# wicstas/pine

Hardware: AMD Instinct MI355X
Metric: Msamples/s (higher is better)
Workload: dtype f32

## Files before the change

pine_amd/csrc/pine_kernels.hip:

```cpp
#include <hip/hip_runtime.h>

#include <climits>
#include <cmath>
#include <cstring>
#include <deque>

#include "pine_plan.h"
#include "pine_bvh_build_device.h"
#include "pine_embree_order.h"
#include "../data/rcpps_table.h"
namespace pine_gpu {

static int device_build(std::vector<BuildPrim>& prims, const std::vector<BuildTask>& roots, FlatAccel& A, int device) {
  int ndev = 0;
  if (hipGetDeviceCount(&ndev) != hipSuccess || device < 0 || device >= ndev) {
    (void)hipGetLastError();
    return -1;
  }
  if (hipSetDevice(device) != hipSuccess) return -1;
  const size_t n = prims.size();
  BuildPrim *d_prims = nullptr, *d_scratch = nullptr;
  BuildTask *d_tasks[2] = {nullptr, nullptr};
  BuildDecision* d_dec = nullptr;
  int *d_rank = nullptr, *d_perm = nullptr, *d_src = nullptr, *d_counts = nullptr;
// ... 203 lines not shown
        } else if (cnt < 0 || ch < 0 || ch >= n_nodes) return bad("child index");
        else todo.push_back({ch, depth + 1});
      }
    }
  }
  for (int i = 0; i < A.top_prim_begin; i++) {
    int tri;
    memcpy(&tri, &A.tri_leaf[size_t(i) * 12 + 9], 4);
    if (tri < 0 || tri >= n_tris) return bad("triangle index of a leaf record");
  }
  for (int i = A.top_prim_begin; i < n_prims; i++)
    if (A.prims[size_t(i)] < 0 || A.prims[size_t(i)] >= int(shapes.size())) return bad("geometry index of a top-level primitive");
  for (const DShape& sh : shapes) {
    if (sh.material < 0 || size_t(sh.material) >= num_materials) return bad("material index");
    if (sh.kind == SHAPE_MESH) {
      int first, count, bvh;
      memcpy(&first, &sh.f[0], 4), memcpy(&count, &sh.f[1], 4), memcpy(&bvh, &sh.f[2], 4);
      if (count > 0 && (bvh < 1 || bvh >= int(A.bvhs.size()) || first < 0 || first + count > n_tris)) return bad("mesh record");
    }
  }
  for (const DLight& L : lights)
    if (L.kind == LIGHT_AREA && (L.geom < 0 || L.geom >= int(shapes.size()))) return bad("area light geometry");
  return 0;
}

}

using namespace pine_gpu;

enum : int { kSpecSourceNone = 0, kSpecSourceCache = 1, kSpecSourceCompiledHere = 2, kSpecSourceBackground = 3 };

namespace pine_gpu {
AbiFingerprint abi_fingerprint() {
  return AbiFingerprint{sizeof(DeviceScene), sizeof(WorkParams), sizeof(Counters), sizeof(DNode), sizeof(DShape), sizeof(DMaterial), sizeof(DLight),
                        offsetof(WorkParams, total_items), offsetof(DeviceScene, cam), kQFields, kQWinDwords, int(QC_WORDS), kQTokenDwords,
                        kTravRecordDwords, kQCtxGlobalDwordsPlain, kQCtxGlobalDwordsSss};
}
}

struct LoadedKernel {
  int device = 0;
  std::string key, image;
  hipModule_t module = nullptr;
  hipFunction_t fn = nullptr;
  ~LoadedKernel() {
    if (module) {
      int keep = 0;
      (void)hipGetDevice(&keep);
      (void)hipSetDevice(device);
      (void)hipModuleUnload(module);
      (void)hipSetDevice(keep);
    }
  }
};
struct LoadedKernels {
  static constexpr size_t kMaxLoaded = 16;
  std::mutex mu;
  std::deque<std::shared_ptr<LoadedKernel>> recent;
  static LoadedKernels& get() {
    static LoadedKernels* q = new LoadedKernels();
    return *q;
  }
  std::shared_ptr<LoadedKernel> find(int device, const std::string& key) {
    std::lock_guard<std::mutex> lock(mu);
    for (auto& k : recent)
      if (k->device == device && k->key == key) return k;
    return nullptr;
  }
  void remember(const std::shared_ptr<LoadedKernel>& k) {
    std::lock_guard<std::mutex> lock(mu);
    recent.push_front(k);
    if (recent.size() > kMaxLoaded) recent.pop_back();
  }
  void forget(const std::string& key) {
    std::lock_guard<std::mutex> lock(mu);
    for (auto it = recent.begin(); it != recent.end();)
      it = (*it)->key == key ? recent.erase(it) : it + 1;
  }
};

constexpr int kUnset = INT_MIN;
struct PlanKnobs {
  int specialize, lds_tris, xstage, trav_min_lanes, trav_min_trips, max_pixels, fair_period, pool_items;
  bool specialize_force, no_lds_scene, mega, no_tile_classes, no_fork, ckpt_every_launch;
  double idle_budget_s;
  int pin_kind, pin_order, lds_nodes_cap;
};
static PlanKnobs read_knobs() {
  auto num = [](const char* name) { return getenv(name) ? atoi(getenv(name)) : kUnset; };
  auto set = [](const char* name) { return getenv(name) != nullptr; };
  const char* kernel = getenv("PINE_GPU_KERNEL");
  const char* budget = getenv("PINE_GPU_IDLE_BUDGET_S");
  const int ckpt = num("PINE_GPU_CKPT_EVERY_LAUNCH");
  int pin_kind = -1, pin_order = -1;
  if (const char* pin = getenv("PINE_GPU_TEST_VARIANT")) {
    const std::string s = pin;
    const size_t colon = s.find(':');
    const std::string kind = s.substr(0, colon), digits = colon == std::string::npos ? "" : s.substr(colon + 1);
    pin_kind = kind == "queue" ? 0 : kind == "mega" ? 1 : 2;
    if (digits.empty() || digits.size() > 6 || digits.find_first_not_of("0123456789") != std::string::npos) pin_kind = 2;
    else pin_order = atoi(digits.c_str());
  }
  return PlanKnobs{num("PINE_GPU_SPECIALIZE"), num("PINE_GPU_LDS_TRIS"), num("PINE_GPU_XSTAGE"), num("PINE_GPU_TRAV_MIN_LANES"),
                   num("PINE_GPU_TRAV_MIN_TRIPS"), num("PINE_GPU_MAX_PIXELS"), num("PINE_GPU_FAIR_PERIOD"), num("PINE_GPU_POOL_ITEMS"),
                   set("PINE_GPU_SPECIALIZE_FORCE"), set("PINE_GPU_NO_LDS_SCENE"), kernel && std::string(kernel) == "mega",
                   set("PINE_GPU_NO_TILE_CLASSES"), set("PINE_GPU_NO_FORK"), ckpt != kUnset && ckpt != 0,
                   budget && atof(budget) > 0 ? atof(budget) : 30.0, pin_kind, pin_order, num("PINE_GPU_TEST_LDS_NODES")};
}

static int plan_adopt_kernel(pine_gpu_plan* p, bool compile_here);
static int plan_specialize(pine_gpu_plan* p, const FlatAccel& A, const std::vector<DShape>& shapes, const std::vector<int>& packed_prims,
                           const pine_gpu_render_params* prm, unsigned need, const PlanKnobs& K) {
  if (K.pin_kind >= 0) return 0;
  bool explicit_want = (prm->flags & PINE_GPU_FLAG_SPECIALIZE) != 0;
  bool automatic = !explicit_want && !(prm->flags & PINE_GPU_FLAG_NO_SPECIALIZE);
  if (K.specialize != kUnset) {
    if (K.specialize != 0) explicit_want = true, automatic = false;
    else explicit_want = automatic = false;
  }
  if ((!explicit_want && !automatic) || p->queue_variant < 0 || (prm->flags & (PINE_GPU_FLAG_FAST | PINE_GPU_FLAG_VERTEX_LOG))) return 0;
  const PineKernelVariant& V = kQueueVariants[p->queue_variant];
  const auto t0 = std::chrono::steady_clock::now();
  const unsigned kLayout = F_LDS_SCENE | F_LDS_TOP | F_LDS_REST | F_XSTAGE | F_SSS;
  unsigned exact = (V.features & kLayout) | need;
  std::string baked;
  if (!(prm->flags & (PINE_GPU_FLAG_SPECIALIZE_NO_BAKE | PINE_GPU_FLAG_ORDER_EMBREE))) {
    if (!(V.features & F_XSTAGE) && A.top_prim_begin == 0) baked = generate_baked_scene(A, shapes, packed_prims);
    else if ((V.features & F_XSTAGE) && A.bvhs.size() == 2) baked = generate_baked_scene(A, shapes, packed_prims, true);
  }
  if (baked.empty() && exact == V.features && !K.specialize_force) return 0;
  if (!baked.empty()) exact |= F_BAKED;
  hipDeviceProp_t prop;
  HIP_OK(hipGetDeviceProperties(&prop, prm->device));
  std::string arch = prop.gcnArchName;
  if (arch.find(':') != std::string::npos) arch = arch.substr(0, arch.find(':'));
  KernelRequest& R = p->spec_request;
  R.baked = baked, R.features = exact, R.ctx = V.ctx, R.arch = arch;
  p->spec_t0 = t0;
  p->spec_explicit = explicit_want;
  std::string err;
  const int found = kernel_cache_lookup(R, err);
  if (found < 0) {
    if (!explicit_want) {
      R = KernelRequest();
      return 0;
    }
    set_error(err);
    return -1;
  }
  if (found == 1) {
    p->spec_source = kSpecSourceCache;
    if (plan_adopt_kernel(p, explicit_want && !(prm->flags & PINE_GPU_FLAG_SPECIALIZE_ASYNC)) == 0) return 0;
    if (explicit_want && !(prm->flags & PINE_GPU_FLAG_SPECIALIZE_ASYNC)) return -1;
    const bool packaged = R.packaged;
    (void)unlink(R.path.c_str());
    const int again = kernel_cache_lookup(R, err, packaged);
    if (again < 0 || (again == 1 && plan_adopt_kernel(p, false) != 0)) {
      p->spec_state.store(kSpecFailed);
      p->spec_async_error = again < 0 ? err : std::string(pine_gpu_last_error());
      return 0;
    }
    if (again == 1) return 0;
  } else if (explicit_want && !(prm->flags & PINE_GPU_FLAG_SPECIALIZE_ASYNC)) {
    p->spec_source = kSpecSourceCompiledHere;
    return plan_adopt_kernel(p, true);
  }
  p->spec_source = kSpecSourceBackground;
  p->spec_job = SpecQueue::get().submit(R, explicit_want);
  if (!p->spec_job) {
    p->spec_state.store(explicit_want ? kSpecFailed : kSpecNone);
    p->spec_async_error = "the background compile queue is full";
    return 0;
  }
  p->spec_state.store(kSpecBuilding);
  return 0;
}

static int plan_adopt_kernel(pine_gpu_plan* p, bool compile_here) {
  KernelRequest& R = p->spec_request;
  bool skip_packaged = false;
  for (int attempt = 0;; attempt++) {
    std::string err;
    const int found = kernel_cache_lookup(R, err, skip_packaged);
    if (found < 0 || (found == 0 && (!compile_here || !kernel_compile(R, err)))) {
      set_error(found == 0 && !compile_here ? "scene specialisation: the code object is not in the cache" : err);
      return -1;
    }
// ... 698 lines not shown
  W.num_local_tiles = (total_tiles - prm->shard_rank + prm->shard_world - 1) / prm->shard_world;
  W.samples_per_item = kspi;
  W.items_per_pixel = spp / kspi;
  W.log2_items_per_pixel = 0;
  while ((1 << W.log2_items_per_pixel) < W.items_per_pixel) W.log2_items_per_pixel++;
  W.tiles_x_magic = unsigned(((1ull << 32) + unsigned(W.tiles_x) - 1) / unsigned(W.tiles_x));
  W.total_items = (unsigned long long)W.num_local_tiles * W.items_per_pixel * 64ull;
  W.tile_order = nullptr;
  W.serial_tiles = 0;
  std::vector<int> serial, free_tiles;
  if (in_path_rng && !uber_rng && kernel.queued() && (kernel.features & F_SSS) != 0 && !K.no_tile_classes && !K.no_fork && spp > 1 &&
      spp_pow2 &&
      tile_classes(H, sp, W, serial, free_tiles) && !free_tiles.empty() && !serial.empty()) {
    p->tile_order = serial;
    p->tile_order.insert(p->tile_order.end(), free_tiles.begin(), free_tiles.end());
    W.serial_tiles = int(serial.size());
    W.samples_per_item = 1;
    W.items_per_pixel = spp;
    W.log2_items_per_pixel = 0;
    while ((1 << W.log2_items_per_pixel) < W.items_per_pixel) W.log2_items_per_pixel++;
    W.total_items = (unsigned long long)W.serial_tiles * 64ull + (unsigned long long)(W.num_local_tiles - W.serial_tiles) * W.items_per_pixel * 64ull;
  }
  if (p->film_w > 65535 || p->film_h > 65535) {
    set_error("film sides above 65535 are not supported");
    return -1;
  }
  W.pass_first_chunk = 0;
  W.pass_chunks = W.items_per_pixel;
  W.pass_chunks_magic = W.pass_chunks > 1 ? unsigned(((1ull << 32) + unsigned(W.pass_chunks) - 1) / unsigned(W.pass_chunks)) : 0u;
  W.pass_row_stride = spp;
  W.free_tile_base = W.serial_tiles;
  W.pass_first_serial_tile = 0;
  if (!plan_passes(W.num_local_tiles, spp, W.samples_per_item, W.serial_tiles, p->pass_samples_req, p->pass_plan)) return -1;
  const PassPlan& PP = p->pass_plan;
  for (int j = 0; j < PP.n; j++)
    if ((PP.rows(j, spp) + unsigned(PP.pass(j, spp).first_sample)) * 64ull >= (1ull << 32)) {
      set_error(PP.n > 1 ? "film pixels x samples of one pass must stay below 2^32 (fewer samples per pass, or several shards)"
                         : "film pixels x samples per pixel of one shard must stay below 2^32 (render in several shards)");
      return -1;
    }
  return 0;
}

static WorkParams pass_work(const pine_gpu_plan* p, int j) {
  WorkParams W = p->W;
  const int spp = p->S.spp;
  const PassPlan::Pass a = p->pass_plan.pass(j, spp);
  if (p->W.items_per_pixel == 1) {
    W.free_tile_base = a.first_tile;
    W.total_items = (unsigned long long)a.tiles * 64ull;
    return W;
  }
  W.serial_tiles = a.tiles;
  W.pass_first_serial_tile = a.first_tile;
  W.free_tile_base = p->W.serial_tiles;
  W.pass_first_chunk = a.first_sample / W.samples_per_item;
  W.pass_chunks = a.samples / W.samples_per_item;
  W.pass_chunks_magic = W.pass_chunks > 1 ? unsigned(((1ull << 32) + unsigned(W.pass_chunks) - 1) / unsigned(W.pass_chunks)) : 0u;
  W.pass_row_stride = a.samples;
  W.total_items = (unsigned long long)a.tiles * 64ull + (unsigned long long)p->pass_plan.free_tiles * unsigned(W.pass_chunks) * 64ull;
  if (p->W.serial_tiles > 0 && a.tiles == 0) {
    W.fork_sealed = 0;
    W.max_pixels = 1 << 20;
  }
  return W;
}

static void schedule_params(pine_gpu_plan* p, const FlatAccel& A, const pine_gpu_render_params* prm, bool uber_rng, const PlanKnobs& K) {
  WorkParams& W = p->W;
  const bool in_path_rng = p->serial_rng;
  W.idle_budget_ticks = (unsigned long long)(K.idle_budget_s * 100e6);
  W.debug_force_bail = (prm->flags & PINE_GPU_FLAG_DEBUG_FORCE_BAIL) ? 1 : 0;
  W.trav_min_lanes = (p->S.lds_nodes > 0 && size_t(p->S.lds_nodes) * 10 >= A.nodes.size() * 9) ? 48 : 0;
  W.trav_min_trips = 8;
  if (!p->spec_request.baked.empty() && (p->spec_request.features & F_XSTAGE)) W.trav_min_trips = 3;
  if (K.trav_min_lanes != kUnset) W.trav_min_lanes = K.trav_min_lanes;
  if (K.trav_min_trips != kUnset) W.trav_min_trips = K.trav_min_trips > 0 ? K.trav_min_trips : 1;
  W.fork_sealed = (in_path_rng && !uber_rng && !K.no_fork) ? 1 : 0;
  W.max_pixels = W.fork_sealed ? 320 : (1 << 20);
  if (K.max_pixels > 0) W.max_pixels = K.max_pixels;
  W.pick_spins = 8;
  W.fair_period = 8;
  if (K.fair_period != kUnset) W.fair_period = K.fair_period;
  W.pool_items = in_path_rng ? 64 : 512;
  if (K.pool_items > 0) W.pool_items = K.pool_items;
  if (W.serial_tiles > 0) W.pool_items = 64;
  W.progress = nullptr;
  W.vertex_log = nullptr;
}

static int size_and_allocate(pine_gpu_plan* p, const pine_gpu_render_params* prm, int spp, const PlanKnobs& K) {
  WorkParams& W = p->W;
  if (prm->flags & PINE_GPU_FLAG_PROGRESS) {
    HIP_OK(hipHostMalloc((void**)&p->h_progress, sizeof(unsigned long long), hipHostMallocMapped));
    *p->h_progress = 0;
    HIP_OK(hipHostGetDevicePointer((void**)&W.progress, p->h_progress, 0));
  }
  hipDeviceProp_t prop;
  HIP_OK(hipGetDeviceProperties(&prop, prm->device));
  int blocks_per_cu = 0;
  const PathKernel kernel = plan_kernel(p);
  if (kernel.queued()) {
    blocks_per_cu = 1;
    HIP_OK(hipFuncSetAttribute(kernel.fn, hipFuncAttributeMaxDynamicSharedMemorySize, int(p->lds_bytes)));
  } else {
    HIP_OK(hipOccupancyMaxActiveBlocksPerMultiprocessor(&blocks_per_cu, kernel.fn, kBlock, p->lds_bytes));
  }
  if (blocks_per_cu < 1) blocks_per_cu = 1;
  if (blocks_per_cu > 8) blocks_per_cu = 8;
  const PassPlan& PP = p->pass_plan;
  unsigned long long launch_items = 0, sample_rows = 0;
  int ckpt_chunks = 0;
  for (int j = 0; j < PP.n; j++) {
    const WorkParams Wj = pass_work(p, j);
    launch_items = std::max(launch_items, Wj.total_items);
    sample_rows = std::max(sample_rows, PP.rows(j, spp));
    ckpt_chunks = std::max(ckpt_chunks, Wj.pass_chunks);
  }
  const unsigned long long want = (launch_items + kernel.ctx - 1) / kernel.ctx;
  p->grid = int(std::min<unsigned long long>(want, (unsigned long long)prop.multiProcessorCount * blocks_per_cu));
  if (p->grid < 1) p->grid = 1;
  if (!p->serial_rng && K.pool_items == kUnset) {
    unsigned long long share = launch_items / ((unsigned long long)p->grid * 32ull);
    int claim = 512;
    while (claim < 2048 && (unsigned long long)claim * 2ull <= share) claim *= 2;
    W.pool_items = claim;
  }

  if (W.items_per_pixel > 1) {
    p->bytes_ckpt = (size_t)(W.num_local_tiles - W.serial_tiles) * ckpt_chunks * 64 * sizeof(ulonglong2);
    HIP_OK(POOL_ALLOC(p->d_ckpt, p->bytes_ckpt));
    if (PP.n > 1) {
      p->bytes_carry = (size_t)PP.free_tiles * 64 * sizeof(ulonglong2);
      HIP_OK(POOL_ALLOC(p->d_rng_carry, p->bytes_carry));
    }
  }
  if (PP.n > 1) {
    HIP_OK(POOL_ALLOC(p->d_sum, (size_t)W.num_local_tiles * 64 * sizeof(float4)));
    p->bytes_carry += (size_t)W.num_local_tiles * 64 * sizeof(float4);
  }
  p->ckpt_every_launch = K.ckpt_every_launch;
  if (!p->tile_order.empty()) {
    HIP_OK(POOL_ALLOC(p->d_tile_order, p->tile_order.size() * sizeof(int)));
    HIP_OK(hipMemcpy(p->d_tile_order, p->tile_order.data(), p->tile_order.size() * sizeof(int), hipMemcpyHostToDevice));
    W.tile_order = p->d_tile_order;
  }
  p->bytes_samples = size_t(sample_rows) * 64 * sizeof(float4);
  HIP_OK(POOL_ALLOC(p->d_samples, p->bytes_samples));
  const size_t fold_slots = size_t(p->grid) * kernel.ctx;
  HIP_OK(POOL_ALLOC(p->d_fold, size_t(prm->max_path_length) * 8 * fold_slots * sizeof(float)));
  if (kernel.queued()) {
    const size_t token_dwords = (kernel.features & F_SSS) ? size_t(p->grid) * (kernel.ctx <= 1024 ? 1024 : 2048) * kQTokenDwords : 0;
    HIP_OK(POOL_ALLOC(p->d_ctxg, (size_t(p->grid) * kernel.ctx * q_ctx_global_dwords(kernel.features) + token_dwords) * sizeof(uint32_t)));
  }
  HIP_OK(POOL_ALLOC(p->d_counters, sizeof(Counters)));
  p->timed = (prm->flags & PINE_GPU_FLAG_TIMING) != 0;
  if (p->timed)
    for (auto& slot : p->ev)
      for (auto& e : slot) HIP_OK(hipEventCreate(&e));
  return 0;
}

static int plan_build(pine_gpu_plan* p, pine_gpu_scene* scene, const pine_gpu_render_params* prm) {
  const PlanKnobs K = read_knobs();
  SceneHost& H = scene_host(scene);
  const int spp = check_params(H, prm);
// ... 566 lines not shown
```

pine_amd/csrc/pine_kernels_device.h:

```cpp
#pragma once
#include <hip/hip_runtime.h>

#include <type_traits>

#include "pine_device.h"

namespace pine_gpu {

constexpr int kBlock = 256;
constexpr int kTile = 8;
#ifndef PINE_LDS_FOLD_LEVELS
#define PINE_LDS_FOLD_LEVELS 1
#endif
constexpr int kLdsFoldLevels = PINE_LDS_FOLD_LEVELS;
constexpr int kPoolItems = 128;
constexpr int kMaxDepth = 32;
constexpr unsigned kFBoxes = F_AABB | F_OBB;
constexpr unsigned kFAnalytic = F_AABB | F_OBB | F_SPHERE | F_DISK | F_CONE | F_UBER;

#ifdef PINE_PROFILE_SECTIONS
static __device__ unsigned long long g_region_lanes[16], g_region_hits[16];
#ifndef PINE_PROFILE_REGIONS
#define REGION(id)
#else
// ... 62 lines not shown
struct SceneView {
  const DShape* leaf;
  const DShape* shapes;
  const DMaterial* materials;
  const DNode* nodes;
  const int* prims;
  const DBvh* bvhs;
  const DLight* lights;
  const float* tri_verts;
  const DNodeOp* node_ops;
  int stack_top;
  int num_shapes;
  const float4* tri_leaf;
  const float* tri_attrs;
  const DNode* lds_nodes;
  int lds_node_count;
  const uint2* lds_tri_entries;
  const float4* lds_tri_verts;
  const EmbreeNode* etree;
  int etree_root;
  const int* emesh;
  int num_emesh;
  const unsigned* rcpps;
};

typedef unsigned int u32x4 __attribute__((ext_vector_type(4)));
typedef __attribute__((address_space(3))) const u32x4 lds_u32x4;
template <unsigned F>
__device__ __forceinline__ DNode fetch_node(const SceneView& S, int index) {
  union {
    DNode n;
    u32x4 q[4];
  } b;
  if constexpr (F & F_LDS_TOP) {
    if (index < S.lds_node_count) {
      lds_u32x4* p = (lds_u32x4*)(S.lds_nodes) + size_t(index) * 4;
      b.q[0] = p[0], b.q[1] = p[1], b.q[2] = p[2], b.q[3] = p[3];
      return b.n;
    }
  }
  const u32x4* g = reinterpret_cast<const u32x4*>(S.nodes + index);
  b.q[0] = g[0], b.q[1] = g[1], b.q[2] = g[2], b.q[3] = g[3];
  return b.n;
}

typedef unsigned int u32x2 __attribute__((ext_vector_type(2)));
typedef __attribute__((address_space(3))) const u32x2 lds_u32x2;
template <unsigned F>
__device__ __forceinline__ void fetch_triangle(const SceneView& S, int i, float (&v)[9], int& tri) {
  if constexpr ((F & F_LDS_TOP) != 0 && (F & F_MESH) != 0) {
    if (S.lds_tri_entries != nullptr) {
      const u32x2 e = *((lds_u32x2*)(S.lds_tri_entries) + i);
      lds_u32x4* vb = (lds_u32x4*)(S.lds_tri_verts);
      const u32x4 a = vb[e.x & 0xffffu], b = vb[e.x >> 16], c = vb[e.y & 0xffffu];
      v[0] = __uint_as_float(a.x), v[1] = __uint_as_float(a.y), v[2] = __uint_as_float(a.z);
      v[3] = __uint_as_float(b.x), v[4] = __uint_as_float(b.y), v[5] = __uint_as_float(b.z);
      v[6] = __uint_as_float(c.x), v[7] = __uint_as_float(c.y), v[8] = __uint_as_float(c.z);
      tri = int(e.y >> 16);
      return;
    }
  }
  const float4* rec = S.tri_leaf + size_t(i) * 3;
  const float4 a = rec[0], b = rec[1], c = rec[2];
  v[0] = a.x, v[1] = a.y, v[2] = a.z, v[3] = a.w, v[4] = b.x, v[5] = b.y, v[6] = b.z, v[7] = b.w, v[8] = c.x;
  tri = __float_as_int(c.y);
}

struct WorkParams {
  int tiles_x, tiles_y;
  int num_local_tiles;
  int shard_rank, shard_world;
  int samples_per_item;
  int items_per_pixel;
  int log2_items_per_pixel;
  unsigned tiles_x_magic;
  unsigned long long total_items;
  const int* tile_order;
  int serial_tiles;
  unsigned long long idle_budget_ticks;
  int debug_force_bail;
  int trav_min_lanes, trav_min_trips;
  int fair_period;
  int pick_spins;
  int pool_items;
  int max_pixels;
  int fork_sealed;
  unsigned long long* progress;
  float* vertex_log;
  int pass_first_chunk;
  int pass_chunks;
  unsigned pass_chunks_magic;
  int pass_row_stride;
  int free_tile_base;
  int pass_first_serial_tile;
};
constexpr int kVertexLogFloats = 16;
__device__ __forceinline__ void post_progress(const WorkParams& W, unsigned long long claimed, unsigned shift) {
  if (W.progress && ((claimed >> shift) & 15ull) == 0ull)
    __hip_atomic_store(W.progress, claimed, __ATOMIC_RELAXED, __HIP_MEMORY_SCOPE_SYSTEM);
}

struct TravLog {
  unsigned* words;
  int n, cap;
  __device__ __forceinline__ void put(unsigned w) {
    if (n < cap) words[n] = w;
    n++;
  }
};
__device__ __forceinline__ float embree_rcp(const unsigned* table, float a) {
  const unsigned u = __float_as_uint(a);
  const int e = int((u >> 23) & 0xffu);
  const unsigned t = table[(u >> 12) & 0x7ffu];
  const int re = int((t >> 23) & 0xffu) + 127 - e;
  const unsigned sign = u & 0x80000000u;
  const float r = __uint_as_float(e == 0 || re >= 255 ? (sign | 0x7f800000u) : re <= 0 ? sign : (sign | (unsigned(re) << 23) | (t & 0x7fffffu)));
  return __fmaf_rn(r, __fmaf_rn(-a, r, 1.0f), r);
}
__device__ __forceinline__ float embree_rcp_safe(const unsigned* table, float a) {
  return embree_rcp(table, fabsf(a) < 1e-18f ? 1e-18f : a);
}
__device__ __forceinline__ bool embree_tri_test(const unsigned* table, const float* v, f3 o, f3 d, float tnear, float tfar, float& t, f2& uv, f3& ng) {
  const f3 v0 = ld3(v), e1 = v0 - ld3(v + 3), e2 = ld3(v + 6) - v0;
  auto crossf = [](f3 a, f3 b) { return f3{__fmaf_rn(a.y, b.z, -(a.z * b.y)), __fmaf_rn(a.z, b.x, -(a.x * b.z)), __fmaf_rn(a.x, b.y, -(a.y * b.x))}; };
  auto dotf = [](f3 a, f3 b) { return __fmaf_rn(a.x, b.x, __fmaf_rn(a.y, b.y, a.z * b.z)); };
  ng = crossf(e2, e1);
  const f3 C = v0 - o, R = crossf(C, d);
  const float den = dotf(ng, d), abs_den = fabsf(den);
  const unsigned sgn = __float_as_uint(den) & 0x80000000u;
  const float U = __uint_as_float(__float_as_uint(dotf(R, e2)) ^ sgn), V = __uint_as_float(__float_as_uint(dotf(R, e1)) ^ sgn);
  if (!(den != 0.0f && U >= 0.0f && V >= 0.0f && U + V <= abs_den)) return false;
  const float T = __uint_as_float(__float_as_uint(dotf(ng, C)) ^ sgn);
  if (!(abs_den * tnear < T && T <= abs_den * tfar)) return false;
  const float r = embree_rcp(table, abs_den);
  t = T * r;
  uv = f2{U * r, V * r};
  return true;
}
__device__ __forceinline__ void mesh_surface_info_embree(const unsigned* table, const float* tri_verts, const float* tri_attrs, int flags, int prim, f3 o, f3 d, DSurface& it) {
  const float* v = tri_verts + size_t(prim) * 9;
  float t = 0.0f;
  f2 bary{0.0f, 0.0f};
  f3 ng = mk3(0.0f);
  (void)embree_tri_test(table, v, o, d, -1.0f, __uint_as_float(0x7f800000u), t, bary, ng);
  it.p = lerp3(bary.x, bary.y, ld3(v), ld3(v + 3), ld3(v + 6));
  it.n = normalize(ng);
  it.uv = bary;
  if (flags != 0) {
    const float* a = tri_attrs + size_t(prim) * 16;
    if (flags & 1) it.n = normalize(lerp3(bary.x, bary.y, ld3(a), ld3(a + 3), ld3(a + 6)));
    if (flags & 2) it.uv = (1.0f - bary.x - bary.y) * f2{a[9], a[10]} + bary.x * f2{a[11], a[12]} + bary.y * f2{a[13], a[14]};
  }
}

template <bool ANY, int STRIDE = kBlock, unsigned F = 0, class StackT = int, bool EMB = false>
__device__ __forceinline__ bool mesh_traverse(const SceneView& S, const DBvh bvh, DRay& ray,
                                              const DRayOct& oct, StackT* stack, int sp0, int& prim_out, TravLog* log = nullptr) {
  bool hit = false;
  auto leaf = [&](int start, int count) -> bool {
    for (int i = start; i < start + count; i++) {
      float v[9];
      int tri;
      fetch_triangle<F>(S, i, v, tri);
      if (log) log->put(0x40000000u | unsigned(tri - bvh.prim_base));
      if constexpr (EMB) {
        float t;
// ... 826 lines not shown
```

pine_amd/csrc/pine_queue_kernel.h:

```cpp
#pragma once


namespace pine_gpu {

#ifndef PINE_QBLOCK
#define PINE_QBLOCK 1024
#endif
constexpr int kQBlock = PINE_QBLOCK;
#ifndef PINE_QCTX
#define PINE_QCTX 1536
#endif
constexpr int kQFields = 12;
enum : int { QS_S = 0, QS_T = 1, QS_W = 2, QS_XS = 3, QS_XC = 4 };
constexpr int q_num_stage_queues(unsigned F) { return ((F & F_LDS_TOP) && (F & F_XSTAGE)) ? 5 : (F & F_SSS) ? 3 : 2; }
constexpr int q_num_queues(unsigned F) { return q_num_stage_queues(F) + ((F & F_SSS) ? 2 : 0); }
enum : int { CF_OX, CF_OY, CF_OZ, CF_DX, CF_DY, CF_DZ, CF_TMAX, CF_ST, CF_PXY, CF_SBASE, CF_GEOM, CF_PRIM };
constexpr unsigned kStFresh = 0xffffffffu;
enum : int { QC_HEAD = 0, QC_TAIL = 8, QC_BUSY = 16, QC_LOCK = 17, QC_EXHAUSTED = 18, QC_PNEXT = 20, QC_PEND = 22, QC_ABORT = 24, QC_PIXELS = 25, QC_WORDS = 32 };
constexpr int kQTokenDwords = 8;
constexpr unsigned kQSpinLimit = 1u << 22;
constexpr int kQWinDwords = 5;

template <int CTX, int NQ = 2, bool ALIAS = false>
struct QLayout {
  static constexpr int ctx = CTX;
  static constexpr int ring = CTX <= 1024 ? 1024 : 2048;
  static constexpr int off_ctl = 0;
  static constexpr int off_ring = off_ctl + QC_WORDS;
  static constexpr int off_state = off_ring + NQ * ring;
  static constexpr int off_sobol = off_state + kQFields * CTX;
  static constexpr int off_win = off_sobol + kLdsSamplerDims * 256 / 4;
  static constexpr int off_stack = ALIAS ? off_win : off_win + kQWinDwords * kQBlock;
  static constexpr size_t fixed_bytes = size_t(off_stack) * 4;
  static constexpr size_t min_stack_bytes = ALIAS ? size_t(kQWinDwords) * kQBlock * 4 : 0;
};

constexpr int kQCtxGlobalDwordsPlain = 4, kQCtxGlobalDwordsSss = 20;
constexpr int q_ctx_trav_offset(unsigned F) { return (F & F_SSS) ? kQCtxGlobalDwordsSss : kQCtxGlobalDwordsPlain; }
constexpr int q_ctx_global_dwords(unsigned F) { return q_ctx_trav_offset(F) + ((F & F_LDS_TOP) ? kTravRecordDwords : 0); }

template <unsigned F, int CTX = PINE_QCTX>
__device__ __forceinline__ void path_queue_body(const DeviceScene& S, const WorkParams& W, const ulonglong2* __restrict__ ckpt, float4* __restrict__ samples,
                                                float* __restrict__ fold, uint32_t* __restrict__ ctxg, Counters* __restrict__ counters) {
  constexpr int kNQ = q_num_queues(F);
  constexpr int kNStage = q_num_stage_queues(F);
  constexpr bool kFork = (F & F_SSS) != 0;
  constexpr bool kVlog = (F & F_VLOG) != 0;
  constexpr int QS_K = kNStage, QS_F = kNStage + 1;
  constexpr bool kTop = (F & F_LDS_TOP) != 0;
  constexpr bool kX = kTop && (F & F_XSTAGE) != 0;
#if defined(PINE_BAKED_SCENE) && !defined(PINE_BAKED_TOP)
  constexpr bool kBaked = true;
  static_assert(!kX, "scenes with meshes are not baked");
  static_assert((F & F_BAKED) != 0, "a baked build instantiates the F_BAKED name");
#else
  constexpr bool kBaked = false;
#endif
  constexpr bool kFlat = kTop && !kBaked;
  static_assert(!(F & F_LDS_REST) || kTop, "F_LDS_REST is an option of the F_LDS_TOP variants");
  static_assert(!(F & F_EMBREE) || (!kTop && !kBaked), "EmbreeAccel's order lives in scene_traverse: not in the flat traversal, not in baked scenes");
  static_assert(!(F & F_XSTAGE) || kTop, "F_XSTAGE is an option of the F_LDS_TOP variants");
  constexpr int kQCtxGlobalDwords = q_ctx_global_dwords(F);
  constexpr int kQCtxTravOffset = q_ctx_trav_offset(F);
  using L = QLayout<CTX, kNQ, kTop>;
  constexpr int kQCtx = L::ctx, kQRing = L::ring, kQOffCtl = L::off_ctl, kQOffRing = L::off_ring, kQOffState = L::off_state,
                kQOffSobol = L::off_sobol, kQOffWin = L::off_win, kQOffStack = L::off_stack;
  extern __shared__ __attribute__((aligned(16))) int lds_raw[];
  typedef const __attribute__((address_space(4))) uint32_t* KargPtr;
  KargPtr kargs = (KargPtr)__builtin_amdgcn_kernarg_segment_ptr();
  asm volatile("" : "+s"(kargs));
  constexpr size_t kWOffset = ((sizeof(DeviceScene) + alignof(WorkParams) - 1) / alignof(WorkParams)) * alignof(WorkParams);
  auto kload = [&](size_t byte_offset, auto* out) {
    uint32_t* o = reinterpret_cast<uint32_t*>(out);
#pragma unroll
    for (size_t i = 0; i < sizeof(*out) / 4; i++) o[i] = kargs[byte_offset / 4 + i];
  };
#define kS(FIELD) ([&] { std::remove_cv_t<decltype(S.FIELD)> v_; kload(offsetof(DeviceScene, FIELD), &v_); return v_; }())
#define kW(FIELD) ([&] { std::remove_cv_t<decltype(W.FIELD)> v_; kload(kWOffset + offsetof(WorkParams, FIELD), &v_); return v_; }())
  constexpr int kSM = kSmLds | ((F & F_SOBOL) ? kSmSobol : 0);
  constexpr bool kBigDim = big_sampler_dimension<F>();
  const unsigned tid = threadIdx.x;
  const unsigned lane = tid & 63;
  unsigned* const qctl = reinterpret_cast<unsigned*>(lds_raw + kQOffCtl);
  unsigned* const ring = reinterpret_cast<unsigned*>(lds_raw + kQOffRing);
  float* const cstf = reinterpret_cast<float*>(lds_raw + kQOffState);
  unsigned* const cstu = reinterpret_cast<unsigned*>(lds_raw + kQOffState);
  using StackT = typename std::conditional<(F & F_LDS_TOP) != 0, unsigned short, int>::type;
  constexpr int kStride = (F & F_LDS_TOP) ? 64 : kQBlock;
  size_t wave_region_bytes = 0;
  if constexpr (F & F_LDS_TOP) {
    wave_region_bytes = size_t(S.stack_total) * 64 * sizeof(StackT);
    if (wave_region_bytes < size_t(kQWinDwords) * 64 * 4) wave_region_bytes = size_t(kQWinDwords) * 64 * 4;
  }
  char* const wave_region = reinterpret_cast<char*>(lds_raw + kQOffStack) + size_t(tid >> 6) * wave_region_bytes;
  StackT* const stack = (F & F_LDS_TOP) ? reinterpret_cast<StackT*>(wave_region) + lane : reinterpret_cast<StackT*>(lds_raw + kQOffStack) + tid;

  {
    const uint4* src = reinterpret_cast<const uint4*>(S.tables.sobol);
    uint4* dst = reinterpret_cast<uint4*>(lds_raw + kQOffSobol);
    for (int i = tid; i < kLdsSamplerDims * 256 / 16; i += kQBlock) dst[i] = src[i];
  }
  SceneView V;
  V.tri_verts = S.tri_verts;
  V.tri_leaf = S.tri_leaf;
  V.tri_attrs = S.tri_attrs;
  V.lds_nodes = nullptr;
  V.lds_node_count = 0;
  V.lds_tri_entries = nullptr;
  V.lds_tri_verts = nullptr;
  V.stack_top = S.stack_top;
  V.num_shapes = S.num_shapes;
  V.etree_root = S.etree_root;
  V.num_emesh = S.num_emesh;
  V.rcpps = reinterpret_cast<const unsigned*>(reinterpret_cast<const char*>(S.blob) + S.off_rcpps);
  V.etree = reinterpret_cast<const EmbreeNode*>(reinterpret_cast<const char*>(S.blob) + S.off_etree);
  V.emesh = reinterpret_cast<const int*>(reinterpret_cast<const char*>(S.blob) + S.off_emesh);
  char* lds_after_stack = nullptr;
  if constexpr (F & F_LDS_TOP) {
    size_t stack_bytes = size_t(S.stack_total) * kQBlock * sizeof(StackT);
    if (stack_bytes < L::min_stack_bytes) stack_bytes = L::min_stack_bytes;
    lds_after_stack = reinterpret_cast<char*>(lds_raw + kQOffStack) + stack_bytes;
    if constexpr (F & F_LDS_REST) lds_after_stack += S.blob_bytes - S.off_shapes;
    if constexpr (F & F_MESH) {
      if (S.lds_tris) {
        const int entry_quads = (S.tri_packet_entries + 1) >> 1, n16 = entry_quads + S.tri_packet_verts;
        uint4* tdst = reinterpret_cast<uint4*>(lds_after_stack);
        for (int i = tid; i < n16; i += kQBlock) tdst[i] = S.tri_packets[i];
        V.lds_tri_entries = reinterpret_cast<const uint2*>(tdst);
        V.lds_tri_verts = reinterpret_cast<const float4*>(tdst + entry_quads);
        lds_after_stack += size_t(n16) * 16;
      }
    }
    uint4* dst = reinterpret_cast<uint4*>(lds_after_stack);
    const uint4* src = reinterpret_cast<const uint4*>(S.nodes);
    for (int i = tid; i < S.lds_nodes * 4; i += kQBlock) dst[i] = src[i];
    V.lds_nodes = reinterpret_cast<const DNode*>(dst);
    V.lds_node_count = S.lds_nodes;
  }
  if constexpr (F & F_LDS_SCENE) {
    static_assert(!(F & F_LDS_TOP), "F_LDS_SCENE already has every node in LDS");
    uint4* dst = reinterpret_cast<uint4*>(lds_raw + kQOffStack + S.stack_total * kQBlock);
// ... 325 lines not shown
                float* r = vlog(cstu[CF_PXY * kQCtx + id], st.s_cur(), st.length());
                r[2] = r[3] = r[4] = 0.0f;
              }
            }
            to_term = true;
          } else {
            if (occluded) {
              float4* q = fold_entry(id, st.length() - 1);
              const float4 e = q[0];
              q[0] = make_float4(0.0f, 0.0f, 0.0f, e.w);
              if (kVlog && W.vertex_log) {
                float* r = vlog(cstu[CF_PXY * kQCtx + id], st.s_cur(), st.length() - 1);
                r[2] = r[3] = r[4] = 0.0f;
              }
            }
            if (flags & kTravClosestResolved) {
              const int geom = int(cstu[CF_GEOM * kQCtx + id]);
              finish_hit(id, geom >= 0, cstf[CF_TMAX * kQCtx + id], geom, 0, st, to_shade, to_term);
            } else {
              to_xc = true;
            }
          }
        } else {
#ifdef PINE_BAKED_TOP
          if (ts.r_next == 1) {
            if (ts.hit_geom != kBakedMeshWord) {
              ray.tmax = __int_as_float(ts.r_pa), ts.hit_geom = ts.r_pan;
            } else if (ts.r_pb && __int_as_float(ts.r_pa) < ray.tmax) {
              DRay rr{ray.o, ray.d, 0.0f, ts.r_pbn ? kFloatMax : kFloatMax * (1.0f - 1e-3f)};
              BakedMesh bm{true, ray.tmax, -1};
              int g = -1;
              const bool hit = scene_traverse_baked_top<false, F, 1>(rr, g, bm);
              ray.tmax = rr.tmax;
              ts.hit_geom = hit ? baked_top_word(g) : -1;
            }
          }
#endif
          finish_hit(id, ts.hit_geom >= 0, ray.tmax, ts.hit_geom, ts.hit_prim, st, to_shade, to_term);
        }
      }
      __builtin_amdgcn_fence(__ATOMIC_RELEASE, "workgroup");
      push2(to_shade, to_term, id);
      if (ANY) push_q(QS_XC, to_xc, id);
      if (retire) id = -1;
      const unsigned long long free_lanes = __ballot(id < 0);
      if (free_lanes != 0) {
        const unsigned h0 = __builtin_amdgcn_readfirstlane(lds_load(&qctl[QC_HEAD + Q]));
        const unsigned avail = __builtin_amdgcn_readfirstlane(lds_load(&qctl[QC_TAIL + Q])) - h0;
        if (avail != 0u) {
          const unsigned nfree = unsigned(__popcll(free_lanes));
          const unsigned want = avail < nfree ? avail : nfree;
          unsigned got = 0;
          if (lane == 0) got = atomicCAS(&qctl[QC_HEAD + Q], h0, h0 + want) == h0 ? 1u : 0u;
          if (__builtin_amdgcn_readfirstlane(got)) {
            const unsigned rank = unsigned(__popcll(free_lanes & ((1ull << lane) - 1ull)));
            if (id < 0 && rank < want) {
              unsigned* slot = &ring[Q * kQRing + ((h0 + rank) & (kQRing - 1))];
              unsigned v, tries = 0;
              while ((v = atomicExch(slot, 0u)) == 0u) {
                if (++tries > kQSpinLimit) {
                  bail(2, unsigned(Q), h0 + rank);
                  break;
                }
                __builtin_amdgcn_s_sleep(1);
              }
              id = int(v) - 1;
              fresh = id >= 0;
            }
            __builtin_amdgcn_fence(__ATOMIC_ACQUIRE, "workgroup");
          }
        }
        if (__ballot(id >= 0) == 0) break;
      }
      if (__builtin_amdgcn_readfirstlane(lds_load(&qctl[QC_ABORT])) != 0u) break;
    }
  };

  unsigned long long idle_since = 0;
#ifdef PINE_PROFILE_SECTIONS
  if (tid == 0) atomicCAS(&counters->t_start, 0ull, wall_clock64());
#endif
  if (kW(debug_force_bail) && blockIdx.x == 0 && tid == 0) bail(7, 0, 0);
  __syncthreads();
  while (true) {
    SEC_MARK(10);
    int stage = -1;
    unsigned n = 0, h = 0;
    bool finished = false;
    {
      auto uload = [&](int w) -> unsigned { return __builtin_amdgcn_readfirstlane(lds_load(&qctl[w])); };
      unsigned hq[kNStage], cq[kNStage];
#pragma unroll
      for (int q = 0; q < kNStage; q++) hq[q] = uload(QC_HEAD + q);
#pragma unroll
      for (int q = 0; q < kNStage; q++) cq[q] = uload(QC_TAIL + q) - hq[q];
      const unsigned busy = uload(QC_BUSY);
      int best = cq[QS_T] > cq[QS_S] ? QS_T : QS_S;
      unsigned cnt_best = cq[best], h_best = hq[best], cnt_all = cq[QS_S] + cq[QS_T];
#pragma unroll
      for (int q = 2; q < kNStage; q++) {
        cnt_all += cq[q];
        if (cq[q] > cnt_best) {
          best = q;
          cnt_best = cq[q];
          h_best = hq[q];
        }
      }
      bool fair_pick = false;
      if constexpr ((F & F_SSS) != 0) {
        const unsigned period = unsigned(W.fair_period < 0 ? -W.fair_period : W.fair_period);
        if (period != 0u && ++pick_no >= period) {
          pick_no = 0;
          if (W.fair_period > 0) {
            if (cq[QS_W] != 0u) {
              best = QS_W;
              cnt_best = cq[QS_W];
              h_best = hq[QS_W];
              fair_pick = true;
            }
          } else {
            unsigned cnt_min = 0xffffffffu;
#pragma unroll
            for (int q = 0; q < kNStage; q++) {
              if (cq[q] != 0u && cq[q] < cnt_min) {
                cnt_min = cq[q];
                best = q;
                h_best = hq[q];
              }
            }
            if (cnt_min != 0xffffffffu) {
              cnt_best = cnt_min;
              fair_pick = true;
            }
          }
        }
      }
      if (cnt_best >= 64u || fair_pick || (cnt_best > 0u && (busy == 0u || spins >= unsigned(W.pick_spins)))) {
        const unsigned h0 = h_best;
        const unsigned want = cnt_best < 64u ? cnt_best : 64u;
        unsigned got = 0;
        if (lane == 0) {
          atomicAdd(&qctl[QC_BUSY], 1u);
          if (atomicCAS(&qctl[QC_HEAD + best], h0, h0 + want) == h0) got = 1;
          else atomicSub(&qctl[QC_BUSY], 1u);
        }
        if (__builtin_amdgcn_readfirstlane(got)) {
          stage = best;
          n = want;
          h = h0;
        }
      } else {
        finished = cnt_all == 0u && busy == 0u;
      }
    }
    if (__builtin_amdgcn_readfirstlane(lds_load(&qctl[QC_ABORT])) != 0u) break;
    if (stage < 0) {
      SEC_MARK(11);
      if (finished) break;
      spins++;
      const unsigned long long now = wall_clock64();
      if (idle_polls++ == 0) idle_since = now;
      if (now - idle_since > kW(idle_budget_ticks)) {
        if (lane == 0)
          bail(1, lds_load(&qctl[QC_BUSY]),
               (lds_load(&qctl[QC_TAIL]) - lds_load(&qctl[QC_HEAD])) | ((lds_load(&qctl[QC_TAIL + 1]) - lds_load(&qctl[QC_HEAD + 1])) << 16));
        break;
      }
      __builtin_amdgcn_s_sleep(4);
      continue;
    }
    spins = 0;
    idle_polls = 0;
    bool valid = lane < n;
    int id = -1;
    if (valid) {
      unsigned* slot = &ring[stage * kQRing + ((h + lane) & (kQRing - 1))];
      unsigned v, tries = 0;
      while ((v = atomicExch(slot, 0u)) == 0u) {
        if (++tries > kQSpinLimit) {
          bail(2, unsigned(stage), h + lane);
          break;
        }
        __builtin_amdgcn_s_sleep(1);
      }
      id = int(v) - 1;
    }
    if (id < 0) valid = false;
    __builtin_amdgcn_fence(__ATOMIC_ACQUIRE, "workgroup");
    SEC_MARK(0);

    if (stage == QS_S) {
      bool to_shade = false, to_term = false, to_walk = false, to_xs = false, to_xc = false;
      bool release = false;
      if (valid) {
        REGION(12);
        const f3 ray_o{cstf[CF_OX * kQCtx + id], cstf[CF_OY * kQCtx + id], cstf[CF_OZ * kQCtx + id]};
        const f3 ray_d{cstf[CF_DX * kQCtx + id], cstf[CF_DY * kQCtx + id], cstf[CF_DZ * kQCtx + id]};
        const float ray_tmax = cstf[CF_TMAX * kQCtx + id];
        PackedState st{cstu[CF_ST * kQCtx + id]};
        const unsigned pxy = cstu[CF_PXY * kQCtx + id];
        const int geom = int(cstu[CF_GEOM * kQCtx + id]) & kPrimIndexMask;
        const int prim = int(cstu[CF_PRIM * kQCtx + id]);
        uint32_t* const cg = ctx_global(id);
        const int wbase = (st.dim() >> 2) < 9 ? (st.dim() >> 2) : 9;
        unsigned* const win = (F & F_LDS_TOP) ? reinterpret_cast<unsigned*>(wave_region) + lane : reinterpret_cast<unsigned*>(lds_raw + kQOffWin) + tid;
        {
          const int pix = int(pxy & 127u) + int((pxy >> 16) & 127u) * 128;
          const uint32_t* rk = reinterpret_cast<const uint32_t*>(S.tables.rank + size_t(pix) * 8) + wbase;
          const uint32_t w0 = rk[0], w1 = rk[1], w2 = rk[2];
          const uint2 sc = *reinterpret_cast<const uint2*>(S.tables.scramble + size_t(pix) * 8);
          win[0] = w0;
          win[kStride] = w1;
          win[2 * kStride] = w2;
          win[3 * kStride] = sc.x;
          win[4 * kStride] = sc.y;
        }
        DTables T = S.tables;
        T.lds_sobol = reinterpret_cast<const uint8_t*>(lds_raw + kQOffSobol);
        T.lds_tile = win - wbase * kStride;
        T.lds_scr = win + 3 * kStride;
        T.tile_stride = kStride;
        T.win_lo = wbase * 4;
        T.win_len = (wbase * 4 + 12 <= kLdsSamplerDims ? 12 : kLdsSamplerDims - wbase * 4);
        DSampler sampler = sampler_of<F>(st, pxy, S.tables.kind, [&] { return int(cg[6]); });
        const int pv_length = st.length();

        const DShape* shape = &V.shapes[geom];
        const DMaterial* mat = &V.materials[shape->material];
        DSurface it;
        hit_surface<F>(V, shape, prim, ray_o, ray_d, ray_tmax, it);
        const f3 wi = -ray_d;
        m3 l2w = coordinate_system(it.n);
        m3 w2l = transpose(l2w);
        const MatParams mp = material_params<F>(mat, V.node_ops, it.p, it.n, it.uv);
        auto rng_load = [&]() -> DRng {
          return DRng{uint64_t(cg[0]) | (uint64_t(cg[1]) << 32), uint64_t(cg[2]) | (uint64_t(cg[3]) << 32)};
        };
        auto rng_store = [&](const DRng& g) {
          cg[0] = uint32_t(g.s0);
          cg[1] = uint32_t(g.s0 >> 32);
          cg[2] = uint32_t(g.s1);
          cg[3] = uint32_t(g.s1 >> 32);
        };
        DBxdf bx;
        choose_lobe<F, kSM>(mat, mp, wi, it.n, st.diffuse_length() > 0, st.walk() != kWalkNone, rng_load, rng_store, T, sampler, bx);
        bx.wi = mul(w2l, wi);
        int beta_channel = 0;
        bool start_walk = false;
        if constexpr (F & F_SSS) {
          if (bx.kind == BX_BSSRDF) {
            float4* const cg4 = reinterpret_cast<float4*>(cg);
            if (st.walk() == kWalkNone) {
              f3 w = -wi;
              if (Refract(wi, it.n, bx.ior, w, nullptr)) {
                DRng g = rng_load();
                const int channel = int(rng_nextf(g) * 3);
                rng_store(g);
                const DRay wr = spawn_ray_raw(it.p, it.n, w);
// ... 430 lines not shown
          kgot = __shfl(kgot, 0);
          wake_more |= __shfl(free_items_left, 0) != 0u;
        }
        if (got == 0 && kgot == 0) {
          if constexpr (kFork) to_free = need_item;
          need_item = false;
          break;
        }
        unsigned rank = __popcll(m & ((1ull << lane) - 1ull));
        if (kFork && need_item && rank < kgot) {
          const unsigned pos = (kbase + rank) & (kQRing - 1);
          unsigned* flag = &ring[QS_K * kQRing + pos];
          unsigned tries = 0;
          while (atomicExch(flag, 0u) == 0u) {
            if (++tries > kQSpinLimit) {
              bail(8, pos, kbase);
              break;
            }
            __builtin_amdgcn_s_sleep(1);
          }
          __builtin_amdgcn_fence(__ATOMIC_ACQUIRE, "workgroup");
          const uint4* tok = reinterpret_cast<const uint4*>(token_slot(pos));
          const uint4 g = tok[0], b = tok[1];
          need_item = false;
          have_path = true;
          pxy = b.x;
          sample_base = b.y;
          s_next = int(b.z);
          item_rng = DRng{uint64_t(g.x) | (uint64_t(g.y) << 32), uint64_t(g.z) | (uint64_t(g.w) << 32)};
          fresh_rng = true;
        }
        rank -= kgot;
        if (need_item && rank < got) {
          const unsigned long long item = base + rank;
          WorkParams Wl;
          kload(kWOffset, &Wl);
          const ItemInfo itf = decode_item(Wl, kS(cam.W), kS(cam.H), kS(spp), item);
          if (itf.valid) {
            need_item = false;
            have_path = true;
            pxy = unsigned(itf.px) | (unsigned(itf.py) << 16);
            sample_base = unsigned(itf.sample_base);
            s_next = itf.chunk * W.samples_per_item;
            DRng g;
            if (itf.serial || W.items_per_pixel == 1) {
              g = rng_seed(hash_pixel(itf.px, itf.py, 0));
            } else {
              const ulonglong2 c = ckpt[itf.ckpt_index];
              g = DRng{c.x, c.y};
            }
            item_rng = g;
            fresh_rng = true;
            if constexpr (kFork) free_item = W.serial_tiles > 0 && !itf.serial;
          } else {
            if constexpr (kFork)
              if (!(W.serial_tiles > 0 && !itf.serial)) atomicSub(&qctl[QC_PIXELS], 1u);
          }
        }
      }
      if constexpr (kFork)
        if (to_free) cstu[CF_ST * kQCtx + id] = kStFresh;
      SEC_MARK(8);
      if (valid && have_path) {
        uint4* cg4 = reinterpret_cast<uint4*>(ctx_global(id));
        DRng g = item_rng;
        if (!fresh_rng)
          g = DRng{uint64_t(rng_words.x) | (uint64_t(rng_words.y) << 32), uint64_t(rng_words.z) | (uint64_t(rng_words.w) << 32)};
        const int px = int(pxy & 0xffffu), py = int(pxy >> 16);
        const DCamera cam = kS(cam);
        const DRay r = camera_sample(cam, px, py, g);
        cg4[0] = make_uint4(uint32_t(g.s0), uint32_t(g.s0 >> 32), uint32_t(g.s1), uint32_t(g.s1 >> 32));
        if constexpr (kBigDim) ctx_global(id)[6] = S.tables.kind == 2 ? 2u : 0u;
        PackedState st{0};
        st.start_sample(s_next);
        if constexpr (kFork)
          if (free_item) st.set_sealed();
        if constexpr (F & F_SOBOL)
          if (S.tables.kind == 2) st.set_dim(2);
        cstu[CF_PXY * kQCtx + id] = pxy;
        cstu[CF_SBASE * kQCtx + id] = sample_base;
        extend(id, r.o, r.d, r.tmax, st, to_shade2, to_term2, to_xc2);
      }
      SEC_MARK(9);
      __builtin_amdgcn_fence(__ATOMIC_RELEASE, "workgroup");
      push2(to_shade2, to_term2, id);
      if constexpr (kX) push_q(QS_XC, to_xc2, id);
      if constexpr (kFork) {
        push_q(QS_F, to_free, id);
        if (wake_more) wake_free(64u);
      }
    }
    if (lane == 0) atomicSub(&qctl[QC_BUSY], 1u);
  }

#ifdef PINE_PROFILE_SECTIONS
  if (tid == 0) atomicMax(&counters->t_end, wall_clock64());
  if (tid == 0 && blockIdx.x < 1024) counters->wg_t[blockIdx.x][2] = wall_clock64();
#endif
  SEC_FLUSH();
  unsigned long long sc = shadow_count;
  for (int off = 32; off > 0; off >>= 1) sc += __shfl_down(sc, off);
  if (lane == 0) atomicAdd(&counters->shadow_rays, sc);
  if constexpr (F & F_SSS) {
    unsigned long long wc = walk_count;
    for (int off = 32; off > 0; off >>= 1) wc += __shfl_down(wc, off);
    if (lane == 0) atomicAdd(&counters->walk_steps, wc);
  }
}

template <unsigned F, int CTX = PINE_QCTX>
__global__ void __launch_bounds__(kQBlock, kQBlock / 256)
path_queue_kernel(DeviceScene S, WorkParams W, const ulonglong2* __restrict__ ckpt, float4* __restrict__ samples,
                  float* __restrict__ fold, uint32_t* __restrict__ ctxg, Counters* __restrict__ counters) {
  path_queue_body<F, CTX>(S, W, ckpt, samples, fold, ctxg, counters);
}

}
```

Measured before the change: 9983.

## Let a wave run on through stage T instead of requeueing terminated lanes

In the queue-based wavefront kernel, when a wave finishes stage T and most lanes would go straight back into T (ids that terminated and were regenerated), the wave now keeps those ids in a per-lane LDS word. It re-runs stage T directly, up to a bound, skipping the queue pick, atomic ring pops and pushes. The goal is to cut queue contention and atomic traffic in the shared LDS scheduler. The cost is that shade-bound lanes are held back for several iterations, and it reuses the wave_region/window LDS as scratch, which could collide with other uses. It is enabled by default, can be disabled by env, and only applies to variants without fork or xstage.

```diff
diff --git a/pine_amd/csrc/pine_kernels.hip b/pine_amd/csrc/pine_kernels.hip
--- a/pine_amd/csrc/pine_kernels.hip
+++ b/pine_amd/csrc/pine_kernels.hip
@@ -309,6 +309,7 @@
 constexpr int kUnset = INT_MIN;
 struct PlanKnobs {
   int specialize, lds_tris, xstage, trav_min_lanes, trav_min_trips, max_pixels, fair_period, pool_items;
+  int t_runon;
   bool specialize_force, no_lds_scene, mega, no_tile_classes, no_fork, ckpt_every_launch;
   double idle_budget_s;
   int pin_kind, pin_order, lds_nodes_cap;
@@ -330,6 +331,7 @@
   }
   return PlanKnobs{num("PINE_GPU_SPECIALIZE"), num("PINE_GPU_LDS_TRIS"), num("PINE_GPU_XSTAGE"), num("PINE_GPU_TRAV_MIN_LANES"),
                    num("PINE_GPU_TRAV_MIN_TRIPS"), num("PINE_GPU_MAX_PIXELS"), num("PINE_GPU_FAIR_PERIOD"), num("PINE_GPU_POOL_ITEMS"),
+                   num("PINE_GPU_T_RUNON"),
                    set("PINE_GPU_SPECIALIZE_FORCE"), set("PINE_GPU_NO_LDS_SCENE"), kernel && std::string(kernel) == "mega",
                    set("PINE_GPU_NO_TILE_CLASSES"), set("PINE_GPU_NO_FORK"), ckpt != kUnset && ckpt != 0,
                    budget && atof(budget) > 0 ? atof(budget) : 30.0, pin_kind, pin_order, num("PINE_GPU_TEST_LDS_NODES")};
@@ -1194,6 +1196,7 @@
   W.pick_spins = 8;
   W.fair_period = 8;
   if (K.fair_period != kUnset) W.fair_period = K.fair_period;
+  W.t_runon = K.t_runon == 0 ? 0 : 1;
   W.pool_items = in_path_rng ? 64 : 512;
   if (K.pool_items > 0) W.pool_items = K.pool_items;
   if (W.serial_tiles > 0) W.pool_items = 64;
diff --git a/pine_amd/csrc/pine_kernels_device.h b/pine_amd/csrc/pine_kernels_device.h
--- a/pine_amd/csrc/pine_kernels_device.h
+++ b/pine_amd/csrc/pine_kernels_device.h
@@ -168,6 +168,7 @@
   int trav_min_lanes, trav_min_trips;
   int fair_period;
   int pick_spins;
+  int t_runon;
   int pool_items;
   int max_pixels;
   int fork_sealed;
diff --git a/pine_amd/csrc/pine_queue_kernel.h b/pine_amd/csrc/pine_queue_kernel.h
--- a/pine_amd/csrc/pine_queue_kernel.h
+++ b/pine_amd/csrc/pine_queue_kernel.h
@@ -20,6 +20,14 @@
 constexpr int kQTokenDwords = 8;
 constexpr unsigned kQSpinLimit = 1u << 22;
 constexpr int kQWinDwords = 5;
+#ifndef PINE_T_RUNON_GATE
+#define PINE_T_RUNON_GATE 64
+#endif
+#ifndef PINE_T_RUNON_BOUND
+#define PINE_T_RUNON_BOUND 8
+#endif
+constexpr int kTRunOnGate = PINE_T_RUNON_GATE, kTRunOnBound = PINE_T_RUNON_BOUND;
+static_assert(kTRunOnGate >= 1 && kTRunOnGate <= 64 && kTRunOnBound >= 1, "stage T's run-on: 1 <= gate <= 64, bound >= 1");
 
 template <int CTX, int NQ = 2, bool ALIAS = false>
 struct QLayout {
@@ -57,6 +65,7 @@
   constexpr bool kBaked = false;
 #endif
   constexpr bool kFlat = kTop && !kBaked;
+  constexpr bool kRunOn = !kFork && !kX && kTRunOnBound > 1;
   static_assert(!(F & F_LDS_REST) || kTop, "F_LDS_REST is an option of the F_LDS_TOP variants");
   static_assert(!(F & F_EMBREE) || (!kTop && !kBaked), "EmbreeAccel's order lives in scene_traverse: not in the flat traversal, not in baked scenes");
   static_assert(!(F & F_XSTAGE) || kTop, "F_XSTAGE is an option of the F_LDS_TOP variants");
@@ -548,12 +557,17 @@
 #endif
   if (kW(debug_force_bail) && blockIdx.x == 0 && tid == 0) bail(7, 0, 0);
   __syncthreads();
+  int held_bodies = 0;
+  constexpr unsigned kHeldTerm = 1u << 30, kHeldShade = 1u << 31;
+  unsigned* const held_word = (F & F_LDS_TOP) ? reinterpret_cast<unsigned*>(wave_region) + lane : reinterpret_cast<unsigned*>(lds_raw + kQOffWin) + tid;
   while (true) {
     SEC_MARK(10);
+    const bool held = kRunOn && held_bodies > 0;
+    const unsigned held_w = held ? *held_word : 0u;
     int stage = -1;
     unsigned n = 0, h = 0;
     bool finished = false;
-    {
+    if (!held) {
       auto uload = [&](int w) -> unsigned { return __builtin_amdgcn_readfirstlane(lds_load(&qctl[w])); };
       unsigned hq[kNStage], cq[kNStage];
 #pragma unroll
@@ -620,6 +634,7 @@
       }
     }
     if (__builtin_amdgcn_readfirstlane(lds_load(&qctl[QC_ABORT])) != 0u) break;
+    if (held) stage = QS_T;
     if (stage < 0) {
       SEC_MARK(11);
       if (finished) break;
@@ -637,9 +652,9 @@
     }
     spins = 0;
     idle_polls = 0;
-    bool valid = lane < n;
-    int id = -1;
-    if (valid) {
+    bool valid = held ? (held_w & kHeldTerm) != 0u : lane < n;
+    int id = held ? int(held_w & ~(kHeldTerm | kHeldShade)) - 1 : -1;
+    if (valid && !held) {
       unsigned* slot = &ring[stage * kQRing + ((h + lane) & (kQRing - 1))];
       unsigned v, tries = 0;
       while ((v = atomicExch(slot, 0u)) == 0u) {
@@ -1236,6 +1251,18 @@
         extend(id, r.o, r.d, r.tmax, st, to_shade2, to_term2, to_xc2);
       }
       SEC_MARK(9);
+      if constexpr (kRunOn) {
+        to_shade2 |= (held_w & kHeldShade) != 0u;
+        if (held_bodies + 1 < kTRunOnBound) {
+          const unsigned long long ma = __ballot(to_term2), md = __ballot(id >= 0 && !to_shade2 && !to_term2);
+          if (ma != 0ull && __popcll(ma | md) >= kTRunOnGate && kW(t_runon) != 0) {
+            held_bodies++;
+            *held_word = unsigned(id + 1) | (to_term2 ? kHeldTerm : 0u) | (to_shade2 ? kHeldShade : 0u);
+            continue;
+          }
+        }
+        held_bodies = 0;
+      }
       __builtin_amdgcn_fence(__ATOMIC_RELEASE, "workgroup");
       push2(to_shade2, to_term2, id);
       if constexpr (kX) push_q(QS_XC, to_xc2, id);
```

Measured after the change: 10210, median of 6. 2.3% higher.
